# AI-sandbox/gnomix

Measured on AMD Instinct MI355X. Metric: haplotypes/sec (+ windows/sec) chr22 7-ancestry inference, higher is better.
Workload: dtype int8 x 7-digit fixed-point weights -> exact i32/i64 logits, f64 sigmoid (logistic base); f32 (tree smoother)

## Files before the change

### gnomix_amd/csrc/gnx_internal.h

```cpp
#pragma once
#include <hip/hip_runtime.h>
#include <stdint.h>
#include <algorithm>
#include <memory>
#include <string>
#include <vector>

#include "../../include/gnomix_hip.h"
#include "gnx_rank_table.h"

struct gnx_devbuf {
  void* p = nullptr;
  size_t cap = 0;
};

struct gnx_prof_pair {
  hipEvent_t a, b;
  int kid;
};

struct gnx_tune {
  int lr_bpc = 0, lr_want = 0;
  int lr_mt = 0, lr_waves = 0;
  int lr_flags = 0;
  int lr_dl = -1;
  int lr_nbuf = 0;
  int p2_mt = 0, p2_cw = 0, p2_ew = 0, p2_xsn = 0, p2_nbuf = 0;
  int p2_decline = 0;
  int lr_p2 = 1;
  int lr_flat = -1;
  int lr_w512 = 0;
  int lr_ws = 0, lr_ws_pw = 2;
  int sm_nw = 0;
  int sm_pair = 1;
  int smf_rpl = 0, smf_nw = 0;
  int crf_impl = 0;
  int crf_flags = 0;
  int forest_threads = 0;
  int forest_wrun = 0;
  int forest_halves = 0;
  int forest_impl = 0;
  int forest_flags = 0;
  int64_t host_batch = 0;
  int h2d_overlap = 1;
  int lr_lds_pad = 0, sm_lds_pad = 0;
  int gnofix_impl = 0;
  int gnofix_aux = 1;
  int gnofix_threads = 0;
  int debug = 0;
};

#define GNX_LDS_OPTIN(bytes, ...)                                                                                  \
  do {                                                                                                             \
    const hipError_t e_optin_ = hipFuncSetAttribute(reinterpret_cast<const void*>(&__VA_ARGS__),                   \
                                                    hipFuncAttributeMaxDynamicSharedMemorySize, (int)(bytes));     \
    if (e_optin_ != hipSuccess) return e_optin_;                                                                   \
  } while (0)

struct gnx_ctx {
  int device = 0;
  gnx_tune tune;
  hipStream_t stream = nullptr;
  bool own_stream = false;
  bool usable = false;
  std::string err;
  int n_cu = 256;
  gnx_devbuf ws_x, ws_b32, ws_b64, ws_p32, ws_p64, ws_lab, ws_misc, ws_scale, ws_bits, ws_lastrow, ws_rpair, ws_y0, ws_cal, ws_marg;
  hipStream_t s_aux = nullptr;
  hipEvent_t ev_aux[2] = {nullptr, nullptr};
  hipStream_t s_in = nullptr, s_out = nullptr;
  hipEvent_t ev_in[2] = {nullptr, nullptr}, ev_done[2] = {nullptr, nullptr}, ev_out[2] = {nullptr, nullptr};
  gnx_devbuf ws_pk, ws_xu, ws_xu2, ws_psi;
  gnx_devbuf ws_rank;
  gnx_devbuf ws_fb, ws_fb_body;
  gnx_devbuf ws_gt2, ws_src, ws_gt2o;
  bool prof = false;
  std::vector<gnx_prof_pair> prof_pending;
  std::vector<hipEvent_t> prof_pool;
  double prof_ms[GNX_K_COUNT] = {0};
  int64_t prof_n[GNX_K_COUNT] = {0};
};

struct BaseLRDev {
  const double* V = nullptr;
  const int8_t* V8 = nullptr;
  const int8_t* V8F = nullptr;
  const double* wscale = nullptr;
  const double* icpt = nullptr;
  const int32_t* chunk_j0 = nullptr;
  const int32_t* chunk_flush0 = nullptr;
  const int32_t* chunk_nflush = nullptr;
  const int32_t* win_chunk0 = nullptr;
  const int32_t* win_chunk1 = nullptr;
  int32_t n_chunks = 0;
  int32_t R = 0;
  int32_t NT = 0;
  int32_t NF = 0;
  int32_t max_piece_chunks = 0;
  const int8_t* V2 = nullptr;
  const int32_t* run_byte = nullptr;
  const int32_t* run_flush0 = nullptr;
  const int32_t* run_nflush = nullptr;
  const int32_t* win_run0 = nullptr;
  const int32_t* win_run1 = nullptr;
  int32_t n_runs = 0;
  int32_t EPR = 0;
  int32_t NT2 = 0;
  const int8_t* V2F = nullptr;
};
constexpr int GNX_LR_FLAT_COLS = 24;
constexpr int GNX_LR_FLAT_TILES = 11;
constexpr int GNX_LR_FLAT_MAX_SPAN = 84;

struct BaseLRLaunch {
  const int8_t* X;
  const int8_t* last_row;
  int64_t N, ldx;
  BaseLRDev d;
  const int32_t* h_win_chunk0;
  const int32_t* h_win_chunk1;
  int32_t W, A, wch;
  int32_t n_htiles;
  int32_t n_rg8;
  int32_t flags;
  int32_t max_chunks;
  int32_t max_wins;
  float* b32;
  double* b64;
  unsigned long long* dbg = nullptr;
};

struct SmoothXGBDev {
  const uint8_t* packed = nullptr;
  const int32_t* group_tree0 = nullptr;
  const int32_t* group_class = nullptr;
  int32_t n_groups = 0, n_trees = 0, D = 0, tree_bytes = 0, max_group = 0;
  float base_score = 0.5f;
  const uint8_t* rk_packed = nullptr;
  const float* rk_thr = nullptr;
  const GnxRankEntry* rk_lut = nullptr;
  const int32_t* rk_group_tree0 = nullptr;
  const int32_t* rk_group_class = nullptr;
  int32_t rk_K = 0, rk_steps = 0, rk_stride = 0, rk_tree_bytes = 0, rk_n_groups = 0, rk_max_group = 0;
  int32_t rk_bits = 0;
  int32_t rk_rpl = 0;
  const uint8_t* h8_packed = nullptr;
  const int32_t* h8_group_tree0 = nullptr;
  const int32_t* h8_group_class = nullptr;
  int32_t h8_tree_bytes = 0, h8_n_groups = 0, h8_max_group = 0;
  const uint8_t* rp_packed = nullptr;
  const int32_t* rp_group_tree0 = nullptr;
  const int32_t* rp_group_class = nullptr;
  int32_t rp_tree_bytes = 0, rp_n_groups = 0, rp_max_group = 0;
  int32_t impl = 0;
  const uint8_t* h3_packed = nullptr;
  const int32_t* h3_group_tree0 = nullptr;
  const int32_t* h3_group_class = nullptr;
  int32_t h3_n_groups = 0, h3_max_group = 0;
  const uint32_t* gf_packed = nullptr;
  int32_t gf_pitch = 0, gf_max_class = 0;
  const uint32_t* bs_nodes = nullptr;
  const float* bs_leaves = nullptr;
  const float* bs_thr = nullptr;
  const uint32_t* bs_lut = nullptr;
  const int32_t* bs_uoff = nullptr;
  const int32_t* bs_binoff = nullptr;
  const int32_t* bs_class_tree0 = nullptr;
  int32_t bs_steps = 0, bs_nbins = 0, bs_wc = 0, bs_nthr = 0, bs_maxbins = 0;
};

struct GnxBsLayout {
  int32_t wp, nr, rw, rb, nbins, hist_bytes, off_cnt, off_hist, off_P, off_bin, off_pi, off_seg, off_wtot, nseg, sl, total;
  uint32_t inv_sl;
};
GnxBsLayout gnx_bs_layout(int A, int S, int wc, int nbins);

__host__ __device__ inline int gnx_gf_tree_words(int D) { return 2 << D; }
constexpr int GNX_GF_PAD_TREES = 24;

constexpr int GNX_H32_WPB = 96;
constexpr int GNX_H32_TREE_BYTES = 320;
constexpr int GNX_H32_MAX_GROUP = 16;
inline size_t gnx_h32_lds_bytes(int A, int S, int G) {
  return (size_t)2 * G * GNX_H32_TREE_BYTES + (size_t)((GNX_H32_WPB + S) / 2) * A * 128;
}
constexpr int GNX_RK_RPL_MAX = 6;

static inline int gnx_tree_bytes(int D) {
  const int half = 1 << (D - 1);
  return ((half * 16 + (half - 1) * 8) + 15) & ~15;
}

#if defined(__HIPCC__)
__device__ __forceinline__ float gnx_walk(const uint8_t* tb, const uint8_t* row, int D) {
  const uint32_t half = 1u << (D - 1);
  uint32_t j = 1;
  for (int d = 0; d < D - 1; ++d) {
    uint2 nd;
    __builtin_memcpy(&nd, tb + half * 16 + (j - 1) * 8, 8);
    float fv;
    __builtin_memcpy(&fv, row + nd.x, 4);
    j = 2 * j + ((fv < __uint_as_float(nd.y)) ? 0u : 1u);
  }
  uint4 n4;
  __builtin_memcpy(&n4, tb + (j - half) * 16, 16);
  float fv;
  __builtin_memcpy(&fv, row + n4.x, 4);
  return (fv < __uint_as_float(n4.y)) ? __uint_as_float(n4.z) : __uint_as_float(n4.w);
}
#endif

struct SmoothXGBLaunch {
  const void* B;
  int32_t b_is_f64;
  int64_t N;
  int32_t W, A, S;
  SmoothXGBDev d;
  float* proba;
  float* marg;
  double* proba64;
  int32_t* labels;
};


struct SmoothCRFLaunch {
  const void* B;
  int32_t b_is_f64;
  int64_t N;
  int32_t W, A;
  const double* state;
  const double* etrans;
  double* psi;
  double* alpha;
  double* scale;
  double* proba64;
  float* proba32;
  int32_t* labels;
  int32_t norm_mask;
};

#ifdef GNX_EXPERIMENTS
hipError_t gnx_launch_smooth_crf_mm(const SmoothCRFLaunch& L, hipStream_t s);
hipError_t gnx_launch_smooth_crf_quad(const SmoothCRFLaunch& L, hipStream_t s);
#endif

struct SmoothCNNLaunch {
  const void* B;
  int32_t b_is_f64;
  int64_t N;
  int32_t W, A, S, reserved;
  const float* weight;
  const float* bias;
  float* proba32;
  double* proba64;
  int32_t* labels;
};

struct SvcWinDev {
  int32_t width, nw, n_sv, g_off;
  int32_t n_ms, poly;
  int64_t sv_off;
  int64_t coef_off;
  int32_t cls_start[36];
  int64_t rv_off;
  double poly_p;
};

struct CovRSKDev {
  const SvcWinDev* win = nullptr;
  const uint32_t* svbits = nullptr;
  const double* coef = nullptr;
  const uint32_t* gtab = nullptr;
  int32_t max_nw = 0, max_width = 0;
  std::vector<int32_t> fast_nw;
};

struct CovRSKLaunch {
  const uint32_t* planes;
  int64_t N, nwp, M;
  int32_t W, A;
  const SvcWinDev* win;
  const uint32_t* svbits;
  const double* coef;
  const uint32_t* gtab;
  int32_t max_nw, max_width;
  float* b32;
  double* b64;
  double* rpair;
  int64_t rpair_haps;
  int64_t n_first, n_count;
  int32_t w_first;
  const int32_t* host_fast_nw;
  hipStream_t aux;
  hipEvent_t ev_fork, ev_join;
  int32_t n_cu;
};

struct GnofixLaunch {
  int8_t* X;
  int64_t ldx, C;
  int32_t x_packed;
  const double* B;
  const int32_t* Y0;
  int32_t* Yout;
  int32_t* n_switches;
  int32_t W, A, S, max_it;
  SmoothXGBDev d;
  const int32_t* class_tree0;
  int32_t bp_in_lds;
  float* bp_scratch;
  uint32_t* hist;
  const uint16_t* R;
  const uint32_t* dif;
  uint32_t* par;
  const uint32_t* gf;
  const float* proba0;
  const float* pmax0;
  const int32_t* order;
  int32_t gf_pitch, gf_cap;
};

struct CalibMaps {
  const int32_t* off;
  const double* x;
  const double* y;
  int32_t thr_f32;
};
struct CalibLaunch {
  const void* in;
  int32_t in_is_f64;
  int64_t R;
  int32_t A;
  const int32_t* off;
  const double* x;
  const double* y;
  int32_t thr_f32;
  double* out64;
  float* out32;
// ... 192 lines not shown
```

### gnomix_amd/csrc/gnx_model_build.hip

```cpp
#include <algorithm>
#include <cmath>
#include <cstdio>
#include <cstdlib>
#include <cstring>
#include <limits>
#include <new>
#include <thread>
#include <utility>

#include "gnx_internal.h"

static inline int fail(gnx_ctx* ctx, int code, const std::string& msg) { return gnx_fail(ctx, code, msg); }

#define HIPCHK(ctx, expr)                                                                      \
  do {                                                                                         \
    hipError_t e__ = (expr);                                                                   \
    if (e__ != hipSuccess)                                                                     \
      return fail((ctx), GNX_EHIP, std::string(#expr) + ": " + hipGetErrorString(e__));        \
  } while (0)

template <typename F>
static unsigned parallel_ranges(size_t n, size_t grain, F&& fn) {
  unsigned nth = std::min<unsigned>(std::max(1u, std::thread::hardware_concurrency()), 16u);
  nth = (unsigned)std::min<size_t>(nth, std::max<size_t>(1, n / std::max<size_t>(grain, 1)));
// ... 430 lines not shown
      ll = d->cond[o + d->left[o + nid]];
      lr = d->cond[o + d->right[o + nid]];
    }
    uint8_t* p = out + (size_t)(j - half) * 16;
    std::memcpy(p, &foff, 4); std::memcpy(p + 4, &thr, 4); std::memcpy(p + 8, &ll, 4); std::memcpy(p + 12, &lr, 4);
    return;
  }
  uint32_t foff = 0;
  float thr = inf;
  if (!leaf) { foff = (uint32_t)d->feat[o + nid] * 4u; thr = d->cond[o + nid]; }
  uint8_t* p = out + (size_t)half * 16 + (size_t)(j - 1) * 8;
  std::memcpy(p, &foff, 4); std::memcpy(p + 4, &thr, 4);
  tree_fill(d, o, leaf ? nid : d->left[o + nid], 2 * j, depth + 1, D, out);
  tree_fill(d, o, leaf ? nid : d->right[o + nid], 2 * j + 1, depth + 1, D, out);
}

static void tree_fill_rk(const gnx_model_desc* d, int32_t o, int32_t nid, uint32_t j, int depth, int D,
                         const std::vector<float>& U, int stride, uint32_t* nodes, float* leaves) {
  const bool leaf = d->left[o + nid] == -1;
  if (depth == D) {
    leaves[j - (1u << D)] = d->cond[o + nid];
    return;
  }
  uint32_t word = 0xFFFFu << 16;
  if (!leaf) {
    const float thr = d->cond[o + nid];
    uint32_t field;
    if (thr != thr || thr == -std::numeric_limits<float>::infinity()) field = 0;
    else if (thr == std::numeric_limits<float>::infinity()) field = 0xFFFFu;
    else field = (uint32_t)(std::lower_bound(U.begin(), U.end(), thr) - U.begin()) + 1u;
    const int f = d->feat[o + nid], A = d->A;
    const uint32_t off = (uint32_t)(((f % A) * stride + f / A) * 2);
    word = (field << 16) | off;
  }
  nodes[j] = word;
  tree_fill_rk(d, o, leaf ? nid : d->left[o + nid], 2 * j, depth + 1, D, U, stride, nodes, leaves);
  tree_fill_rk(d, o, leaf ? nid : d->right[o + nid], 2 * j + 1, depth + 1, D, U, stride, nodes, leaves);
}

static int build_xgb_rk(gnx_model* m, const gnx_model_desc* d, const std::vector<int32_t>& order, int D) {
  const char* impl = std::getenv("GNX_SMOOTH_IMPL");
  if (impl && std::string(impl) == "f32") return GNX_OK;
  const int A = d->A, S = d->S;
  std::vector<float> U;
  for (int t = 0; t < d->n_trees; ++t)
    for (int32_t k = d->tree_off[t]; k < d->tree_off[t + 1]; ++k)
      if (d->left[k] != -1 && std::isfinite(d->cond[k])) U.push_back(d->cond[k]);
  std::sort(U.begin(), U.end());
  U.erase(std::unique(U.begin(), U.end()), U.end());
  const int nseg = (int)((d->C / d->M + 63) / 64);
  int rpl = 1;
  if (nseg >= 2) {
    int best_waste = 1 << 30;
    for (int r : {3, 2, 4}) {
      const int waste = (nseg + r - 1) / r * r - nseg;
      if (waste < best_waste) { best_waste = waste; rpl = r; }
    }
  }
  if (const char* e = std::getenv("GNX_RK_RPL")) rpl = std::max(1, std::min(GNX_RK_RPL_MAX, std::atoi(e)));
  int stride = rpl * 64 + S - 1;
  stride += stride & 1;
  if (U.size() > 65000 || (size_t)A * stride * 2 > 65535) return GNX_OK;
  if (U.empty()) U.push_back(0.5f);
  const int K = (int)U.size();
  GnxRankTable rt;
  gnx_rank_table_build(U, std::getenv("GNX_RK_BITS") ? std::atoi(std::getenv("GNX_RK_BITS")) : 0, rt);
  const std::vector<GnxRankEntry>& lut = rt.lut;
  const int steps = rt.steps;
  const int tree_bytes = 8 << D;
  int group_bytes = 4096;
  if (const char* e = std::getenv("GNX_RK_GROUP_BYTES")) group_bytes = std::max(tree_bytes, std::min(8192, std::atoi(e)));
  const int G = std::max(1, group_bytes / tree_bytes);
  std::vector<int32_t> group_tree0, group_class;
  {
    int in_group = 0, cur = -1;
    for (size_t k = 0; k < order.size(); ++k) {
      const int c = d->tree_class[order[k]];
      if (c != cur || in_group == G) { group_tree0.push_back((int32_t)k); group_class.push_back(c); in_group = 0; cur = c; }
      ++in_group;
    }
    group_tree0.push_back((int32_t)order.size());
  }
  std::vector<uint8_t> packed(order.size() * (size_t)tree_bytes, 0);
  for (size_t k = 0; k < order.size(); ++k) {
    uint8_t* tb = packed.data() + k * tree_bytes;
    tree_fill_rk(d, d->tree_off[order[k]], 0, 1, 0, D, U, stride, reinterpret_cast<uint32_t*>(tb),
                 reinterpret_cast<float*>(tb + ((size_t)4 << D)));
  }
  int rc;
  if ((rc = gnx_dev_upload(m, packed, &m->xgb.rk_packed, 64)) != GNX_OK) return rc;
  if ((rc = gnx_dev_upload(m, U, &m->xgb.rk_thr, 64)) != GNX_OK) return rc;
  if ((rc = gnx_dev_upload(m, lut, &m->xgb.rk_lut)) != GNX_OK) return rc;
  if ((rc = gnx_dev_upload(m, group_tree0, &m->xgb.rk_group_tree0)) != GNX_OK) return rc;
  if ((rc = gnx_dev_upload(m, group_class, &m->xgb.rk_group_class)) != GNX_OK) return rc;
  m->xgb.rk_K = K; m->xgb.rk_bits = rt.bits; m->xgb.rk_steps = steps; m->xgb.rk_stride = stride; m->xgb.rk_tree_bytes = tree_bytes;
  m->xgb.rk_n_groups = (int32_t)group_class.size(); m->xgb.rk_max_group = G; m->xgb.rk_rpl = rpl;
#ifdef GNX_EXPERIMENTS
  m->xgb.impl = (impl && std::string(impl) == "h64") ? 2 : (impl && std::string(impl) == "rk") ? 1 : 3;
#else
  m->xgb.impl = (impl && std::string(impl) == "rk") ? 1 : 3;
#endif
  if ((size_t)A * (2 * S + 2) * 2 <= 65535) {
    const int pitch = 2 * S + 2;
    const size_t tw = (size_t)gnx_gf_tree_words(D);
    std::vector<uint32_t> gf((order.size() + GNX_GF_PAD_TREES) * tw, 0u);
    for (size_t k = 0; k < order.size(); ++k) {
      uint32_t* tb = gf.data() + k * tw;
      tree_fill_rk(d, d->tree_off[order[k]], 0, 1, 0, D, U, pitch, tb, reinterpret_cast<float*>(tb + ((size_t)1 << D)));
    }
    if ((rc = gnx_dev_upload(m, gf, &m->xgb.gf_packed, 64)) != GNX_OK) return rc;
    std::vector<int> cnt(A, 0);
    int mc = 0;
    for (size_t k = 0; k < order.size(); ++k) mc = std::max(mc, ++cnt[d->tree_class[order[k]]]);
    m->xgb.gf_pitch = pitch; m->xgb.gf_max_class = mc;
  }
  if (D >= 2 && D <= 6) {
    const int tbp = 12 << D;
    const int Gp = std::max(2, (4096 / tbp) & ~1);
    std::vector<int32_t> gp_tree0, gp_class;
    {
      int in_group = 0, cur = -1;
      for (size_t k = 0; k < order.size(); ++k) {
        const int c = d->tree_class[order[k]];
        if (c != cur || in_group == Gp) { gp_tree0.push_back((int32_t)k); gp_class.push_back(c); in_group = 0; cur = c; }
        ++in_group;
      }
      gp_tree0.push_back((int32_t)order.size());
    }
    std::vector<uint8_t> pp(order.size() * (size_t)tbp, 0);
    std::vector<uint32_t> nodes((size_t)1 << D);
    std::vector<float> leaves((size_t)1 << D);
    size_t g = 0;
    for (size_t k = 0; k < order.size(); ++k) {
      while ((size_t)gp_tree0[g + 1] <= k) ++g;
      const uint32_t base = (uint32_t)(k - (size_t)gp_tree0[g]) * (uint32_t)tbp;
      std::fill(nodes.begin(), nodes.end(), 0u);
      tree_fill_rk(d, d->tree_off[order[k]], 0, 1, 0, D, U, stride, nodes.data(), leaves.data());
      uint32_t* o = reinterpret_cast<uint32_t*>(pp.data() + k * tbp);
      auto kids = [&](uint32_t j) {
        const uint32_t l = 2 * j < (1u << D) ? base + 8u * (2 * j) : base + (8u << D) + 4u * (2 * j - (1u << D));
        const uint32_t step = 2 * j < (1u << D) ? 8u : 4u;
        return l | ((l + step) << 16);
      };
      for (uint32_t j = 2; j < (1u << D); ++j) { o[2 * j] = nodes[j]; o[2 * j + 1] = kids(j); }
      o[0] = nodes[2]; o[1] = nodes[3]; o[2] = nodes[1]; o[3] = kids(2);
      memcpy(pp.data() + k * tbp + ((size_t)8 << D), leaves.data(), sizeof(float) << D);
    }
    if ((rc = gnx_dev_upload(m, pp, &m->xgb.rp_packed, 64)) != GNX_OK) return rc;
    if ((rc = gnx_dev_upload(m, gp_tree0, &m->xgb.rp_group_tree0)) != GNX_OK) return rc;
    if ((rc = gnx_dev_upload(m, gp_class, &m->xgb.rp_group_class)) != GNX_OK) return rc;
    m->xgb.rp_tree_bytes = tbp; m->xgb.rp_n_groups = (int32_t)gp_class.size(); m->xgb.rp_max_group = Gp;
  }
  if (D == 4 && ((size_t)(S >> 1) * A + A) * 128 <= 65536) {
    constexpr int tb3 = GNX_H32_TREE_BYTES;
    int G3 = 2;
    {
      const size_t strip = gnx_h32_lds_bytes(A, S, 0);
      if (strip + 4 * (size_t)tb3 <= (size_t)80 * 1024) G3 = std::min(GNX_H32_MAX_GROUP, (int)((((size_t)80 * 1024 - strip) / 2) / tb3) & ~1);
    }
    std::vector<int32_t> g3_tree0, g3_class;
    {
      int in_group = 0, cur = -1;
      for (size_t k = 0; k < order.size(); ++k) {
        const int c = d->tree_class[order[k]];
        if (c != cur || in_group == G3) { g3_tree0.push_back((int32_t)k); g3_class.push_back(c); in_group = 0; cur = c; }
        ++in_group;
      }
      g3_tree0.push_back((int32_t)order.size());
    }
    std::vector<uint8_t> p3(order.size() * (size_t)tb3, 0);
    std::vector<uint32_t> nodes(16);
    std::vector<float> leaves(16);
    size_t g = 0;
    for (size_t k = 0; k < order.size(); ++k) {
      while ((size_t)g3_tree0[g + 1] <= k) ++g;
      const uint32_t base = (uint32_t)(k - (size_t)g3_tree0[g]) * (uint32_t)tb3;
      std::fill(nodes.begin(), nodes.end(), 0u);
      tree_fill_rk(d, d->tree_off[order[k]], 0, 1, 0, 4, U, stride, nodes.data(), leaves.data());
      for (uint32_t odd = 0; odd < 2; ++odd) {
        const uint32_t nb = base + odd * 192u;
        uint32_t* o = reinterpret_cast<uint32_t*>(p3.data() + k * tb3 + odd * 192u);
        auto w0 = [&](uint32_t j) {
          const uint32_t hw = (nodes[j] & 0xffffu) / 2, a = hw / (uint32_t)stride, s = hw - a * (uint32_t)stride + odd;
          return (nodes[j] & 0xffff0000u) | (((s >> 1) * (uint32_t)A + a) * 128u + (s & 1u) * 2u);
        };
        auto kids = [&](uint32_t j) {
          const uint32_t l = 2 * j < 16u ? nb + 8u * (2 * j) : base + 128u + 4u * (2 * j - 16u);
          const uint32_t step = 2 * j < 16u ? 8u : 4u;
          return l | ((l + step) << 16);
        };
        for (uint32_t j = 2; j < 16u; ++j) { o[2 * j] = w0(j); o[2 * j + 1] = kids(j); }
        o[0] = w0(2); o[1] = w0(3); o[2] = w0(1); o[3] = kids(2);
      }
      memcpy(p3.data() + k * tb3 + 128, leaves.data(), 64);
    }
    if ((rc = gnx_dev_upload(m, p3, &m->xgb.h3_packed, 64)) != GNX_OK) return rc;
    if ((rc = gnx_dev_upload(m, g3_tree0, &m->xgb.h3_group_tree0)) != GNX_OK) return rc;
    if ((rc = gnx_dev_upload(m, g3_class, &m->xgb.h3_group_class)) != GNX_OK) return rc;
    m->xgb.h3_n_groups = (int32_t)g3_class.size(); m->xgb.h3_max_group = G3;
    if (!impl || !*impl) m->xgb.impl = 6;
    else if (std::string(impl) == "h32") m->xgb.impl = 5;
  }
#ifdef GNX_EXPERIMENTS
  if (D >= 2 && D <= 6 && (size_t)S * A < 65536) {
    const int tb8 = 12 << D;
    int G8 = std::max(4, (4096 / tb8) & ~3);
    {
      const size_t strip16 = (size_t)(16 * 3 + S - 1) * A * 128;
      if (strip16 + 2 * (size_t)G8 * tb8 <= (size_t)160 * 1024) {
        int per_class = 0;
        std::vector<int> cnt(A, 0);
        for (size_t k = 0; k < order.size(); ++k) per_class = std::max(per_class, ++cnt[d->tree_class[order[k]]]);
        const int fit = (int)((((size_t)160 * 1024 - strip16) / 2) / tb8) & ~3;
        G8 = std::max(G8, std::min({fit, (32768 / tb8) & ~3, (per_class + 3) & ~3}));
      }
    }
    std::vector<int32_t> g8_tree0, g8_class;
    {
      int in_group = 0, cur = -1;
      for (size_t k = 0; k < order.size(); ++k) {
        const int c = d->tree_class[order[k]];
        if (c != cur || in_group == G8) { g8_tree0.push_back((int32_t)k); g8_class.push_back(c); in_group = 0; cur = c; }
        ++in_group;
      }
      g8_tree0.push_back((int32_t)order.size());
    }
    std::vector<uint8_t> p8(order.size() * (size_t)tb8, 0);
    std::vector<uint32_t> nodes((size_t)1 << D);
    std::vector<float> leaves((size_t)1 << D);
    size_t g = 0;
    for (size_t k = 0; k < order.size(); ++k) {
      while ((size_t)g8_tree0[g + 1] <= k) ++g;
      const uint32_t base = (uint32_t)(k - (size_t)g8_tree0[g]) * (uint32_t)tb8;
      std::fill(nodes.begin(), nodes.end(), 0u);
      tree_fill_rk(d, d->tree_off[order[k]], 0, 1, 0, D, U, stride, nodes.data(), leaves.data());
      for (uint32_t j = 1; j < (1u << D); ++j) {
        const uint32_t h = (nodes[j] & 0xffffu) / 2, a = h / (uint32_t)stride, sidx = h - a * (uint32_t)stride;
        nodes[j] = (nodes[j] & 0xffff0000u) | (sidx * (uint32_t)A + a);
      }
      uint32_t* o = reinterpret_cast<uint32_t*>(p8.data() + k * tb8);
      auto kids = [&](uint32_t j) {
        const uint32_t l = 2 * j < (1u << D) ? base + 8u * (2 * j) : base + (8u << D) + 4u * (2 * j - (1u << D));
        const uint32_t step = 2 * j < (1u << D) ? 8u : 4u;
        return l | ((l + step) << 16);
      };
      for (uint32_t j = 2; j < (1u << D); ++j) { o[2 * j] = nodes[j]; o[2 * j + 1] = kids(j); }
      o[0] = nodes[2]; o[1] = nodes[3]; o[2] = nodes[1]; o[3] = kids(2);
      memcpy(p8.data() + k * tb8 + ((size_t)8 << D), leaves.data(), sizeof(float) << D);
    }
    if ((rc = gnx_dev_upload(m, p8, &m->xgb.h8_packed, 64)) != GNX_OK) return rc;
    if ((rc = gnx_dev_upload(m, g8_tree0, &m->xgb.h8_group_tree0)) != GNX_OK) return rc;
    if ((rc = gnx_dev_upload(m, g8_class, &m->xgb.h8_group_class)) != GNX_OK) return rc;
    m->xgb.h8_tree_bytes = tb8; m->xgb.h8_n_groups = (int32_t)g8_class.size(); m->xgb.h8_max_group = G8;
  }
#endif
  return GNX_OK;
}

#ifdef GNX_EXPERIMENTS
static void tree_fill_bs(const gnx_model_desc* d, int32_t o, int32_t nid, uint32_t j, int depth, const std::vector<std::vector<float>>& Uc,
                         const std::vector<int32_t>& binoff, const GnxBsLayout& Y, uint32_t* words, float* leaves) {
  const bool leaf = d->left[o + nid] == -1;
  if (depth == 4) {
    leaves[j - 16u] = d->cond[o + nid];
    return;
  }
  uint32_t a = 0, kf = 0, sw = 0;
  if (!leaf) {
    const float thr = d->cond[o + nid];
    const int f = d->feat[o + nid], A = d->A;
    a = (uint32_t)(f % A);
    sw = (uint32_t)(f / A);
    const std::vector<float>& U = Uc[a];
    if (thr != thr || thr == -std::numeric_limits<float>::infinity()) kf = 0;
    else if (thr == std::numeric_limits<float>::infinity()) kf = (uint32_t)U.size() + 1u;
    else kf = (uint32_t)(std::lower_bound(U.begin(), U.end(), thr) - U.begin()) + 1u;
  }
  const uint32_t cnt_addr = (uint32_t)Y.off_cnt + (uint32_t)binoff[a] + kf;
  words[2 * j] = (sw & 31u) | (cnt_addr << 16);
  words[2 * j + 1] = (uint32_t)Y.off_P + a * (uint32_t)(Y.nr * Y.rb) + (sw >> 5) * 4u;
  tree_fill_bs(d, o, leaf ? nid : d->left[o + nid], 2 * j, depth + 1, Uc, binoff, Y, words, leaves);
  tree_fill_bs(d, o, leaf ? nid : d->right[o + nid], 2 * j + 1, depth + 1, Uc, binoff, Y, words, leaves);
}

static int build_xgb_bs(gnx_model* m, const gnx_model_desc* d, const std::vector<int32_t>& order, int D) {
  const char* impl = std::getenv("GNX_SMOOTH_IMPL");
  if (impl && std::string(impl) == "f32") return GNX_OK;
  const int A = d->A, S = d->S;
  if (D > 4 || A > 16) return GNX_OK;
  std::vector<std::vector<float>> Uc((size_t)A);
  for (int t = 0; t < d->n_trees; ++t)
    for (int32_t k = d->tree_off[t]; k < d->tree_off[t + 1]; ++k)
      if (d->left[k] != -1 && std::isfinite(d->cond[k])) Uc[(size_t)(d->feat[k] % A)].push_back(d->cond[k]);
  std::vector<int32_t> uoff((size_t)A + 1, 0), binoff((size_t)A + 1, 0);
  std::vector<float> U;
  for (int c = 0; c < A; ++c) {
    std::vector<float>& u = Uc[(size_t)c];
    std::sort(u.begin(), u.end());
    u.erase(std::unique(u.begin(), u.end()), u.end());
    if (u.empty()) u.push_back(0.5f);
    if (u.size() > 60000) return GNX_OK;
    U.insert(U.end(), u.begin(), u.end());
    uoff[(size_t)c + 1] = (int32_t)U.size();
    binoff[(size_t)c + 1] = binoff[(size_t)c] + (((int32_t)u.size() + 2 + 15) & ~15);
  }
  const int nbins = binoff[(size_t)A];
  if (nbins > 65000) return GNX_OK;
  int wc = 128;
  if (wc + S - 1 > 255 || gnx_bs_layout(A, S, wc, nbins).total > 160 * 1024) return GNX_OK;
  const GnxBsLayout Y = gnx_bs_layout(A, S, wc, nbins);
  std::vector<uint32_t> lut((size_t)A * 1024);
  int steps = 0;
  for (int c = 0; c < A; ++c) {
    const std::vector<float>& u = Uc[(size_t)c];
    const int K = (int)u.size();
    for (int b = 0; b < 1024; ++b) {
      const int lo = b == 0 ? 0 : (int)(std::lower_bound(u.begin(), u.end(), (float)b / 1024.0f) - u.begin());
      const int hi = b == 1023 ? K : (int)(std::lower_bound(u.begin(), u.end(), (float)(b + 1) / 1024.0f) - u.begin());
      lut[(size_t)c * 1024 + (size_t)b] = (uint32_t)lo | ((uint32_t)hi << 16);
      int st = 0;
      while ((1 << st) < hi - lo + 1) ++st;
      steps = std::max(steps, st);
    }
  }
  std::vector<uint32_t> nodes(order.size() * 32, 0u);
  std::vector<float> leaves(order.size() * 16, 0.f);
  for (size_t k = 0; k < order.size(); ++k)
    tree_fill_bs(d, d->tree_off[order[k]], 0, 1, 0, Uc, binoff, Y, nodes.data() + k * 32, leaves.data() + k * 16);
  std::vector<int32_t> ct0((size_t)A + 1, 0);
  for (int t = 0; t < d->n_trees; ++t) ct0[(size_t)d->tree_class[t] + 1] += 1;
  for (int c = 0; c < A; ++c) ct0[(size_t)c + 1] += ct0[(size_t)c];
  int rc;
  if ((rc = gnx_dev_upload(m, nodes, &m->xgb.bs_nodes, 128)) != GNX_OK) return rc;
  if ((rc = gnx_dev_upload(m, leaves, &m->xgb.bs_leaves, 64)) != GNX_OK) return rc;
  if ((rc = gnx_dev_upload(m, U, &m->xgb.bs_thr, 64)) != GNX_OK) return rc;
  if ((rc = gnx_dev_upload(m, lut, &m->xgb.bs_lut)) != GNX_OK) return rc;
  if ((rc = gnx_dev_upload(m, uoff, &m->xgb.bs_uoff)) != GNX_OK) return rc;
  if ((rc = gnx_dev_upload(m, binoff, &m->xgb.bs_binoff)) != GNX_OK) return rc;
  if ((rc = gnx_dev_upload(m, ct0, &m->xgb.bs_class_tree0)) != GNX_OK) return rc;
  m->xgb.bs_steps = steps; m->xgb.bs_nbins = nbins; m->xgb.bs_wc = wc; m->xgb.bs_nthr = (int32_t)U.size();
  for (int c = 0; c < A; ++c) m->xgb.bs_maxbins = std::max(m->xgb.bs_maxbins, binoff[(size_t)c + 1] - binoff[(size_t)c]);
  if (impl && std::string(impl) == "bs") m->xgb.impl = 4;
  return GNX_OK;
}
#endif

int gnx_build_xgb(gnx_model* m, const gnx_model_desc* d) {
  gnx_ctx* ctx = m->ctx;
  const int A = d->A, S = d->S, F = S * A;
  if (d->n_trees <= 0 || !d->tree_off || !d->left || !d->right || !d->feat || !d->cond || !d->tree_class)
    return fail(ctx, GNX_EINVAL, "xgb smoother: tree arrays missing");
  const int64_t W = d->C / d->M;
// ... 385 lines not shown
```

### gnomix_amd/csrc/k_smooth_xgb_h32.hip

```cpp
#include <cstdio>
#include <cstdlib>

#include "gnx_internal.h"
#include "gnx_exp.h"
#include "gnx_rank.h"

namespace {

constexpr int HB = 32;
constexpr int RW = 3;
constexpr int NWAVE = 16;
constexpr int WPW = 2 * RW;
constexpr int WPB = NWAVE * WPW;
constexpr int THREADS = NWAVE * 64;
constexpr int TB = GNX_H32_TREE_BYTES;
static_assert(WPB == GNX_H32_WPB, "the model loader sizes the staging groups for this block");

#if defined(__HIP_DEVICE_COMPILE__)
template <typename T>
__device__ __forceinline__ const __attribute__((address_space(3))) T* lds_at(uint32_t a) {
  return (const __attribute__((address_space(3))) T*)(uintptr_t)a;
}
#else
template <typename T>
__device__ const T* lds_at(uint32_t) { return nullptr; }
#endif
typedef uint32_t u32x2 __attribute__((ext_vector_type(2)));
typedef uint32_t u32x4 __attribute__((ext_vector_type(4)));
__device__ __forceinline__ uint32_t step_ptr(uint32_t w0, uint32_t w1, uint32_t r) {
  uint32_t p;
  asm("v_cmp_le_u32_sdwa vcc, %[n], %[r] src0_sel:WORD_1 src1_sel:DWORD\n\t"
      "v_cndmask_b32_sdwa %[p], %[w], %[w], vcc dst_sel:DWORD dst_unused:UNUSED_PAD src0_sel:WORD_0 src1_sel:WORD_1"
      : [p] "=v"(p)
      : [n] "v"(w0), [r] "v"(r), [w] "v"(w1)
      : "vcc");
  return p;
}
__device__ __forceinline__ void first_ptr(uint32_t root, uint32_t r, uint32_t l0, uint32_t r0, uint32_t l1, uint32_t r1, uint32_t& w0,
                                          uint32_t& w1) {
  asm("v_cmp_le_u32_sdwa vcc, %[n], %[r] src0_sel:WORD_1 src1_sel:DWORD\n\t"
      "v_cndmask_b32 %[x], %[l0], %[r0], vcc\n\t"
      "v_cndmask_b32 %[y], %[l1], %[r1], vcc"
      : [x] "=&v"(w0), [y] "=&v"(w1)
      : [n] "v"(root), [r] "v"(r), [l0] "v"(l0), [r0] "v"(r0), [l1] "v"(l1), [r1] "v"(r1)
      : "vcc");
}

template <int NT>
__device__ __forceinline__ void walk_h32(uint32_t tb, const uint32_t* rb, float* psum) {
  constexpr int NC = NT * RW;
  uint32_t w0[NC], w1[NC], r[NC], p[NC];
  u32x4 top[NT];
#pragma unroll
  for (int t = 0; t < NT; ++t) top[t] = *lds_at<u32x4>(tb + t * TB);
  constexpr uint32_t SIB = 16u * 0x10001u;
#pragma unroll
  for (int c = 0; c < NC; ++c) r[c] = *lds_at<uint16_t>(rb[c % RW] + (top[c / RW].z & 0xffffu));
#pragma unroll
  for (int c = 0; c < NC; ++c)
    first_ptr(top[c / RW].z, r[c], top[c / RW].x, top[c / RW].y, top[c / RW].w, top[c / RW].w + SIB, w0[c], w1[c]);
#pragma unroll
  for (int c = 0; c < NC; ++c) r[c] = *lds_at<uint16_t>(rb[c % RW] + (w0[c] & 0xffffu));
#pragma unroll
  for (int c = 0; c < NC; ++c) p[c] = step_ptr(w0[c], w1[c], r[c]);
#pragma unroll
  for (int d = 2; d < 4; ++d) {
#pragma unroll
    for (int c = 0; c < NC; ++c) {
      const u32x2 nd = *lds_at<u32x2>(p[c]);
      w0[c] = nd.x;
      w1[c] = nd.y;
    }
#pragma unroll
    for (int c = 0; c < NC; ++c) r[c] = *lds_at<uint16_t>(rb[c % RW] + (w0[c] & 0xffffu));
#pragma unroll
    for (int c = 0; c < NC; ++c) p[c] = step_ptr(w0[c], w1[c], r[c]);
  }
  float lf[NC];
#pragma unroll
  for (int c = 0; c < NC; ++c) lf[c] = *lds_at<float>(p[c]);
#pragma unroll
  for (int t = 0; t < NT; ++t)
#pragma unroll
    for (int k = 0; k < RW; ++k) psum[k] += lf[t * RW + k];
}

__global__ __launch_bounds__(THREADS, 8) void k_smooth_xgb_h32(SmoothXGBLaunch L, int gw) {
  extern __shared__ __attribute__((aligned(16))) uint8_t lds[];
  const int A = L.A, W = L.W, S = L.S, pad = (S + 1) / 2;
  const int buf_bytes = L.d.h3_max_group * TB;
  const int P = WPB + S - 1;
  uint8_t* tbuf0 = lds;
  uint8_t* tbuf1 = tbuf0 + buf_bytes;
  uint8_t* strip = tbuf1 + buf_bytes;
  const int tid = threadIdx.x, lane = tid & 63, wave = tid >> 6, h = lane & 31, hv = lane >> 5;
  const int64_t hb = blockIdx.y, h0 = hb * HB;
  const int w0 = blockIdx.x * WPB;

  {
    constexpr int NV = 4;
    const int per_h = P * A;
    const int hl = (wave & 1) * 16 + (lane >> 2);
    const size_t row = (size_t)min(h0 + hl, L.N - 1) * W;
    const int dq = 32 / A, da = 32 - dq * A;
    int rr = (wave >> 1) * 4 + (lane & 3);
    int q = rr / A, a = rr - q * A;
    const bool interior = w0 >= pad && w0 + P <= pad + W;
    const size_t run0 = (row + (size_t)(interior ? w0 - pad : 0)) * A;
    for (; rr < per_h; rr += NV * 32) {
      float p[NV];
      uint32_t r[NV];
      int dst[NV];
      bool ok[NV];
      if (interior) {
#pragma unroll
        for (int i = 0; i < NV; ++i) {
          ok[i] = rr + i * 32 < per_h;
          const size_t idx = run0 + (size_t)min(rr + i * 32, per_h - 1);
          p[i] = L.b_is_f64 ? (float)reinterpret_cast<const double*>(L.B)[idx] : reinterpret_cast<const float*>(L.B)[idx];
          dst[i] = ((q >> 1) * A + a) * 128 + hl * 4 + (q & 1) * 2;
          a += da;
          q += dq;
          if (a >= A) { a -= A; ++q; }
        }
      } else {
#pragma unroll
        for (int i = 0; i < NV; ++i) {
          ok[i] = rr + i * 32 < per_h;
          const int qc = ok[i] ? q : P - 1, ac = ok[i] ? a : A - 1;
          const int j = min(w0 + qc, W + 2 * pad - 1);
          const size_t idx = (row + slide_src(j, W, pad)) * A + ac;
          p[i] = L.b_is_f64 ? (float)reinterpret_cast<const double*>(L.B)[idx] : reinterpret_cast<const float*>(L.B)[idx];
          dst[i] = ((qc >> 1) * A + ac) * 128 + hl * 4 + (qc & 1) * 2;
          a += da;
          q += dq;
          if (a >= A) { a -= A; ++q; }
        }
      }
      ranks<NV>(L.d.rk_thr, L.d.rk_lut, L.d.rk_K, L.d.rk_bits, L.d.rk_steps, p, r);
#pragma unroll
      for (int i = 0; i < NV; ++i)
        if (ok[i]) *reinterpret_cast<uint16_t*>(strip + dst[i]) = (uint16_t)r[i];
    }
  }

  const int64_t n = h0 + h;
  uint32_t rb[RW];
  bool valid[RW];
#pragma unroll
  for (int k = 0; k < RW; ++k) {
    rb[k] = (uint32_t)(uintptr_t)strip + (uint32_t)(((wave * RW + k) * A) * 128 + h * 4);
    valid[k] = (n < L.N) && (w0 + wave * WPW + 2 * k + hv < W);
  }
  const size_t cls_stride = (size_t)gridDim.y * W * HB;
  float* mrow = L.marg + ((size_t)hb * W + w0 + wave * WPW + hv) * HB + h;

  const int ng = L.d.h3_n_groups;
  uint4 stg;
#define GNX_G_LOAD(g)                                                                               \
  {                                                                                                 \
    const int t0_ = L.d.h3_group_tree0[g], t1_ = L.d.h3_group_tree0[(g) + 1];                       \
    const int last_ = (t1_ - t0_) * TB / 16 - 1;                                                    \
    stg = reinterpret_cast<const uint4*>(L.d.h3_packed + (size_t)t0_ * TB)[min(tid, last_)];        \
  }
#define GNX_G_STORE(dst)                                                                            \
  {                                                                                                 \
     \
    const int pc_ = (tid * 16 % TB) >> 4;                                                           \
    const bool node_ = pc_ < 8 || pc_ >= 12;                                                        \
    const uint32_t add_ = node_ ? (uint32_t)(uintptr_t)(dst) * 0x10001u : 0u;                       \
    stg.w += add_;                                                                                  \
    stg.y += (pc_ == 0 || pc_ == 12) ? 0u : add_;                                                   \
    if (tid * 16 < buf_bytes) *reinterpret_cast<uint4*>((dst) + (size_t)tid * 16) = stg;            \
  }
  float psum[RW];
#pragma unroll
  for (int k = 0; k < RW; ++k) psum[k] = 0.f;

  GNX_G_LOAD(0);
  GNX_G_STORE(tbuf0);
  __syncthreads();

  int cur_class = L.d.h3_group_class[0];
  for (int g = 0; g < ng; ++g) {
    uint8_t* cur = (g & 1) ? tbuf1 : tbuf0;
    uint8_t* nxt = (g & 1) ? tbuf0 : tbuf1;
    const int gn = min(g + 1, ng - 1);
    GNX_G_LOAD(gn);
    const int cls = L.d.h3_group_class[g];
    if (cls != cur_class) {
#pragma unroll
      for (int k = 0; k < RW; ++k) {
        if (valid[k]) mrow[(size_t)cur_class * cls_stride + (size_t)(2 * k) * HB] = L.d.base_score + psum[k];
        psum[k] = 0.f;
      }
      cur_class = cls;
    }
    const int nt = L.d.h3_group_tree0[g + 1] - L.d.h3_group_tree0[g];
    const uint32_t tb = (uint32_t)(uintptr_t)cur + (uint32_t)hv * 192u;
    int t = 0;
    for (; t + 2 <= nt; t += 2) walk_h32<2>(tb + (uint32_t)t * TB, rb, psum);
    for (; t < nt; ++t) walk_h32<1>(tb + (uint32_t)t * TB, rb, psum);
    GNX_G_STORE(nxt);
    __syncthreads();
  }
#undef GNX_G_LOAD
#undef GNX_G_STORE
#pragma unroll
  for (int k = 0; k < RW; ++k)
    if (valid[k]) mrow[(size_t)cur_class * cls_stride + (size_t)(2 * k) * HB] = L.d.base_score + psum[k];

  float* tile = reinterpret_cast<float*>(lds);
  const int rowlen = gw * WPW * A, pitch = rowlen | 1;
  for (int g0 = 0; g0 < NWAVE; g0 += gw) {
    if (wave >= g0 && wave < g0 + gw) {
#pragma unroll
      for (int k = 0; k < RW; ++k) {
        if (!valid[k]) continue;
        const float* mg = mrow + (size_t)(2 * k) * HB;
        float* o = tile + (size_t)h * pitch + ((wave - g0) * WPW + 2 * k + hv) * A;
        float wmax = mg[0];
        for (int a = 1; a < A; ++a) wmax = fmaxf(mg[(size_t)a * cls_stride], wmax);
        double wsum = 0.0;
        for (int a = 0; a < A; ++a) {
          const float e = gnx_softmax_exp(mg[(size_t)a * cls_stride] - wmax);
          o[a] = e;
          wsum += (double)e;
        }
        const float fs = (float)wsum;
        for (int a = 0; a < A; ++a) o[a] = o[a] / fs;
      }
    }
    __syncthreads();
    const int wb = w0 + g0 * WPW;
    for (int e = tid; e < HB * rowlen; e += THREADS) {
      const int hl = e / rowlen, c = e - hl * rowlen;
      const int64_t nn = h0 + hl;
      if (nn < L.N && wb + c / A < W) {
        const float p = tile[(size_t)hl * pitch + c];
        const size_t idx = ((size_t)nn * W + wb) * A + c;
        L.proba[idx] = p;
        if (L.proba64) L.proba64[idx] = (double)p;
      }
    }
    if (L.labels) {
      const int nwl = gw * WPW;
      for (int e = tid; e < HB * nwl; e += THREADS) {
        const int hl = e / nwl, wl = e - hl * nwl;
        const int64_t nn = h0 + hl;
        if (nn < L.N && wb + wl < W) {
          const float* o = tile + (size_t)hl * pitch + wl * A;
          int best = 0;
          float bv = -1.f;
          for (int a = 0; a < A; ++a) {
            const float p = o[a];
            if (p > bv) { bv = p; best = a; }
          }
          L.labels[(size_t)nn * W + wb + wl] = best;
        }
      }
    }
    __syncthreads();
  }
}

size_t lds_need(const SmoothXGBDev& d, int A, int S) { return gnx_h32_lds_bytes(A, S, d.h3_max_group); }

}

bool gnx_smooth_h32_fits(const SmoothXGBDev& d, int A, int S) {
  return d.h3_packed && d.rk_thr && d.D == 4 && lds_need(d, A, S) <= (size_t)80 * 1024;
}

hipError_t gnx_launch_smooth_xgb_h32(const SmoothXGBLaunch& L, hipStream_t s) {
  if (L.N <= 0) return hipSuccess;
  if (!gnx_smooth_h32_fits(L.d, L.A, L.S)) return hipErrorInvalidValue;
  const size_t lds = lds_need(L.d, L.A, L.S);
  int gw = NWAVE;
  while (gw > 1 && (size_t)HB * ((size_t)(gw * WPW * L.A) | 1) * 4 > lds) gw >>= 1;
  if ((size_t)HB * ((size_t)(gw * WPW * L.A) | 1) * 4 > lds) return hipErrorInvalidValue;
  const dim3 grid((unsigned)((L.W + WPB - 1) / WPB), (unsigned)((L.N + HB - 1) / HB));
  GNX_LDS_OPTIN(lds, k_smooth_xgb_h32);
  hipLaunchKernelGGL(k_smooth_xgb_h32, grid, dim3(THREADS), lds, s, L, gw);
  return hipGetLastError();
}
```

Baseline: 3.731 million.

## Prebake LDS addresses into fixed-size h32 tree groups and skip dead waves

Tree packing moves to a shared header and pads each tree group to a fixed G-tree buffer. Child addresses are now baked at build time against absolute LDS offsets that alternate between two buffers. This removes the per-group address patching during staging and the loads of group start indices, and the staging load becomes a single strided read. Waves whose windows lie past the edge skip the tree walks, and the strip size uses only the live window count. The change relies on dynamic LDS starting at address zero (checked at runtime) and adds compile-time ablation switches, with some host memory spent on padding.

```diff
diff --git a/gnomix_amd/csrc/gnx_h32_layout.h b/gnomix_amd/csrc/gnx_h32_layout.h
--- /dev/null
+++ b/gnomix_amd/csrc/gnx_h32_layout.h
@@ -0,0 +1,75 @@
+#pragma once
+#include <stdint.h>
+#include <string.h>
+
+#include <algorithm>
+#include <vector>
+
+#if defined(__HIPCC__)
+#define GNX_H32_HD __host__ __device__ __forceinline__
+#else
+#define GNX_H32_HD inline
+#endif
+
+constexpr int GNX_H32_WPB = 96;
+constexpr int GNX_H32_TREE_BYTES = 320;
+constexpr int GNX_H32_MAX_GROUP = 16;
+
+GNX_H32_HD uint32_t gnx_h32_buf_bytes(int G) { return (uint32_t)G * (uint32_t)GNX_H32_TREE_BYTES; }
+GNX_H32_HD uint32_t gnx_h32_group_lds(int g, int G) { return (uint32_t)(g & 1) * gnx_h32_buf_bytes(G); }
+inline size_t gnx_h32_lds_bytes(int A, int S, int G) {
+  return (size_t)2 * gnx_h32_buf_bytes(G) + (size_t)((GNX_H32_WPB + S) / 2) * A * 128;
+}
+inline int gnx_h32_group_trees(int A, int S) {
+  const size_t strip = gnx_h32_lds_bytes(A, S, 0), tb = GNX_H32_TREE_BYTES;
+  if (strip + 4 * tb > (size_t)80 * 1024) return 2;
+  return std::min(GNX_H32_MAX_GROUP, (int)((((size_t)80 * 1024 - strip) / 2) / tb) & ~1);
+}
+
+struct GnxH32Pack {
+  int G = 0;
+  std::vector<int32_t> tree0, cls;
+  std::vector<uint8_t> packed;
+};
+
+inline void gnx_h32_pack(const std::vector<int>& cls, const std::vector<uint32_t>& nodes, const std::vector<float>& leaves, int A,
+                         int S, int stride, GnxH32Pack& out) {
+  constexpr uint32_t TB = GNX_H32_TREE_BYTES;
+  const int G = gnx_h32_group_trees(A, S);
+  out.G = G;
+  out.tree0.clear();
+  out.cls.clear();
+  {
+    int in_group = 0, cur = -1;
+    for (size_t k = 0; k < cls.size(); ++k) {
+      if (cls[k] != cur || in_group == G) { out.tree0.push_back((int32_t)k); out.cls.push_back(cls[k]); in_group = 0; cur = cls[k]; }
+      ++in_group;
+    }
+    out.tree0.push_back((int32_t)cls.size());
+  }
+  out.packed.assign(out.cls.size() * (size_t)gnx_h32_buf_bytes(G), 0);
+  size_t g = 0;
+  for (size_t k = 0; k < cls.size(); ++k) {
+    while ((size_t)out.tree0[g + 1] <= k) ++g;
+    const uint32_t in_group = (uint32_t)(k - (size_t)out.tree0[g]);
+    const uint32_t base = gnx_h32_group_lds((int)g, G) + in_group * TB;
+    uint8_t* tree = out.packed.data() + g * (size_t)gnx_h32_buf_bytes(G) + (size_t)in_group * TB;
+    const uint32_t* nd = nodes.data() + 16 * k;
+    for (uint32_t odd = 0; odd < 2; ++odd) {
+      const uint32_t nb = base + odd * 192u;
+      uint32_t* o = reinterpret_cast<uint32_t*>(tree + odd * 192u);
+      auto w0 = [&](uint32_t j) {
+        const uint32_t hw = (nd[j] & 0xffffu) / 2, a = hw / (uint32_t)stride, s = hw - a * (uint32_t)stride + odd;
+        return (nd[j] & 0xffff0000u) | (((s >> 1) * (uint32_t)A + a) * 128u + (s & 1u) * 2u);
+      };
+      auto kids = [&](uint32_t j) {
+        const uint32_t l = 2 * j < 16u ? nb + 8u * (2 * j) : base + 128u + 4u * (2 * j - 16u);
+        const uint32_t step = 2 * j < 16u ? 8u : 4u;
+        return l | ((l + step) << 16);
+      };
+      for (uint32_t j = 2; j < 16u; ++j) { o[2 * j] = w0(j); o[2 * j + 1] = kids(j); }
+      o[0] = w0(2); o[1] = w0(3); o[2] = w0(1); o[3] = kids(2);
+    }
+    memcpy(tree + 128, leaves.data() + 16 * k, 64);
+  }
+}
diff --git a/gnomix_amd/csrc/gnx_internal.h b/gnomix_amd/csrc/gnx_internal.h
--- a/gnomix_amd/csrc/gnx_internal.h
+++ b/gnomix_amd/csrc/gnx_internal.h
@@ -8,6 +8,7 @@
 
 #include "../../include/gnomix_hip.h"
 #include "gnx_rank_table.h"
+#include "gnx_h32_layout.h"
 
 struct gnx_devbuf {
   void* p = nullptr;
@@ -178,12 +179,6 @@
 __host__ __device__ inline int gnx_gf_tree_words(int D) { return 2 << D; }
 constexpr int GNX_GF_PAD_TREES = 24;
 
-constexpr int GNX_H32_WPB = 96;
-constexpr int GNX_H32_TREE_BYTES = 320;
-constexpr int GNX_H32_MAX_GROUP = 16;
-inline size_t gnx_h32_lds_bytes(int A, int S, int G) {
-  return (size_t)2 * G * GNX_H32_TREE_BYTES + (size_t)((GNX_H32_WPB + S) / 2) * A * 128;
-}
 constexpr int GNX_RK_RPL_MAX = 6;
 
 static inline int gnx_tree_bytes(int D) {
diff --git a/gnomix_amd/csrc/gnx_model_build.hip b/gnomix_amd/csrc/gnx_model_build.hip
--- a/gnomix_amd/csrc/gnx_model_build.hip
+++ b/gnomix_amd/csrc/gnx_model_build.hip
@@ -606,52 +606,19 @@
     m->xgb.rp_tree_bytes = tbp; m->xgb.rp_n_groups = (int32_t)gp_class.size(); m->xgb.rp_max_group = Gp;
   }
   if (D == 4 && ((size_t)(S >> 1) * A + A) * 128 <= 65536) {
-    constexpr int tb3 = GNX_H32_TREE_BYTES;
-    int G3 = 2;
-    {
-      const size_t strip = gnx_h32_lds_bytes(A, S, 0);
-      if (strip + 4 * (size_t)tb3 <= (size_t)80 * 1024) G3 = std::min(GNX_H32_MAX_GROUP, (int)((((size_t)80 * 1024 - strip) / 2) / tb3) & ~1);
-    }
-    std::vector<int32_t> g3_tree0, g3_class;
-    {
-      int in_group = 0, cur = -1;
-      for (size_t k = 0; k < order.size(); ++k) {
-        const int c = d->tree_class[order[k]];
-        if (c != cur || in_group == G3) { g3_tree0.push_back((int32_t)k); g3_class.push_back(c); in_group = 0; cur = c; }
-        ++in_group;
-      }
-      g3_tree0.push_back((int32_t)order.size());
-    }
-    std::vector<uint8_t> p3(order.size() * (size_t)tb3, 0);
-    std::vector<uint32_t> nodes(16);
-    std::vector<float> leaves(16);
-    size_t g = 0;
+    std::vector<int> cls3(order.size());
+    std::vector<uint32_t> nodes(order.size() * 16, 0u);
+    std::vector<float> leaves(order.size() * 16, 0.f);
     for (size_t k = 0; k < order.size(); ++k) {
-      while ((size_t)g3_tree0[g + 1] <= k) ++g;
-      const uint32_t base = (uint32_t)(k - (size_t)g3_tree0[g]) * (uint32_t)tb3;
-      std::fill(nodes.begin(), nodes.end(), 0u);
-      tree_fill_rk(d, d->tree_off[order[k]], 0, 1, 0, 4, U, stride, nodes.data(), leaves.data());
-      for (uint32_t odd = 0; odd < 2; ++odd) {
-        const uint32_t nb = base + odd * 192u;
-        uint32_t* o = reinterpret_cast<uint32_t*>(p3.data() + k * tb3 + odd * 192u);
-        auto w0 = [&](uint32_t j) {
-          const uint32_t hw = (nodes[j] & 0xffffu) / 2, a = hw / (uint32_t)stride, s = hw - a * (uint32_t)stride + odd;
-          return (nodes[j] & 0xffff0000u) | (((s >> 1) * (uint32_t)A + a) * 128u + (s & 1u) * 2u);
-        };
-        auto kids = [&](uint32_t j) {
-          const uint32_t l = 2 * j < 16u ? nb + 8u * (2 * j) : base + 128u + 4u * (2 * j - 16u);
-          const uint32_t step = 2 * j < 16u ? 8u : 4u;
-          return l | ((l + step) << 16);
-        };
-        for (uint32_t j = 2; j < 16u; ++j) { o[2 * j] = w0(j); o[2 * j + 1] = kids(j); }
-        o[0] = w0(2); o[1] = w0(3); o[2] = w0(1); o[3] = kids(2);
-      }
-      memcpy(p3.data() + k * tb3 + 128, leaves.data(), 64);
-    }
-    if ((rc = gnx_dev_upload(m, p3, &m->xgb.h3_packed, 64)) != GNX_OK) return rc;
-    if ((rc = gnx_dev_upload(m, g3_tree0, &m->xgb.h3_group_tree0)) != GNX_OK) return rc;
-    if ((rc = gnx_dev_upload(m, g3_class, &m->xgb.h3_group_class)) != GNX_OK) return rc;
-    m->xgb.h3_n_groups = (int32_t)g3_class.size(); m->xgb.h3_max_group = G3;
+      cls3[k] = d->tree_class[order[k]];
+      tree_fill_rk(d, d->tree_off[order[k]], 0, 1, 0, 4, U, stride, nodes.data() + 16 * k, leaves.data() + 16 * k);
+    }
+    GnxH32Pack pk;
+    gnx_h32_pack(cls3, nodes, leaves, A, S, stride, pk);
+    if ((rc = gnx_dev_upload(m, pk.packed, &m->xgb.h3_packed, 64)) != GNX_OK) return rc;
+    if ((rc = gnx_dev_upload(m, pk.tree0, &m->xgb.h3_group_tree0)) != GNX_OK) return rc;
+    if ((rc = gnx_dev_upload(m, pk.cls, &m->xgb.h3_group_class)) != GNX_OK) return rc;
+    m->xgb.h3_n_groups = (int32_t)pk.cls.size(); m->xgb.h3_max_group = pk.G;
     if (!impl || !*impl) m->xgb.impl = 6;
     else if (std::string(impl) == "h32") m->xgb.impl = 5;
   }
diff --git a/gnomix_amd/csrc/k_smooth_xgb_h32.hip b/gnomix_amd/csrc/k_smooth_xgb_h32.hip
--- a/gnomix_amd/csrc/k_smooth_xgb_h32.hip
+++ b/gnomix_amd/csrc/k_smooth_xgb_h32.hip
@@ -5,8 +5,13 @@
 #include "gnx_exp.h"
 #include "gnx_rank.h"
 
+#ifndef GNX_H32_ABLATE
+#define GNX_H32_ABLATE 0
+#endif
+
 namespace {
 
+constexpr bool ABL_GROUPS = (GNX_H32_ABLATE & 3) != 0, ABL_BARRIER = (GNX_H32_ABLATE & 2) != 0;
 constexpr int HB = 32;
 constexpr int RW = 3;
 constexpr int NWAVE = 16;
@@ -24,6 +29,11 @@
 #else
 template <typename T>
 __device__ const T* lds_at(uint32_t) { return nullptr; }
+#endif
+#if defined(__HIP_DEVICE_COMPILE__)
+__device__ __forceinline__ int wave_uniform(int v) { return __builtin_amdgcn_readfirstlane(v); }
+#else
+__device__ int wave_uniform(int v) { return v; }
 #endif
 typedef uint32_t u32x2 __attribute__((ext_vector_type(2)));
 typedef uint32_t u32x4 __attribute__((ext_vector_type(4)));
@@ -88,14 +98,14 @@
 __global__ __launch_bounds__(THREADS, 8) void k_smooth_xgb_h32(SmoothXGBLaunch L, int gw) {
   extern __shared__ __attribute__((aligned(16))) uint8_t lds[];
   const int A = L.A, W = L.W, S = L.S, pad = (S + 1) / 2;
-  const int buf_bytes = L.d.h3_max_group * TB;
-  const int P = WPB + S - 1;
-  uint8_t* tbuf0 = lds;
-  uint8_t* tbuf1 = tbuf0 + buf_bytes;
-  uint8_t* strip = tbuf1 + buf_bytes;
+  const int G = L.d.h3_max_group;
+  const int buf_bytes = (int)gnx_h32_buf_bytes(G);
+  uint8_t* strip = lds + 2 * buf_bytes;
   const int tid = threadIdx.x, lane = tid & 63, wave = tid >> 6, h = lane & 31, hv = lane >> 5;
   const int64_t hb = blockIdx.y, h0 = hb * HB;
   const int w0 = blockIdx.x * WPB;
+  const int live = min(WPB, W - w0);
+  const int P = live + S - 1;
 
   {
     constexpr int NV = 4;
@@ -156,37 +166,22 @@
   float* mrow = L.marg + ((size_t)hb * W + w0 + wave * WPW + hv) * HB + h;
 
   const int ng = L.d.h3_n_groups;
-  uint4 stg;
-#define GNX_G_LOAD(g)                                                                               \
-  {                                                                                                 \
-    const int t0_ = L.d.h3_group_tree0[g], t1_ = L.d.h3_group_tree0[(g) + 1];                       \
-    const int last_ = (t1_ - t0_) * TB / 16 - 1;                                                    \
-    stg = reinterpret_cast<const uint4*>(L.d.h3_packed + (size_t)t0_ * TB)[min(tid, last_)];        \
-  }
-#define GNX_G_STORE(dst)                                                                            \
-  {                                                                                                 \
-     \
-    const int pc_ = (tid * 16 % TB) >> 4;                                                           \
-    const bool node_ = pc_ < 8 || pc_ >= 12;                                                        \
-    const uint32_t add_ = node_ ? (uint32_t)(uintptr_t)(dst) * 0x10001u : 0u;                       \
-    stg.w += add_;                                                                                  \
-    stg.y += (pc_ == 0 || pc_ == 12) ? 0u : add_;                                                   \
-    if (tid * 16 < buf_bytes) *reinterpret_cast<uint4*>((dst) + (size_t)tid * 16) = stg;            \
-  }
+  const uint32_t lds0 = (uint32_t)(uintptr_t)lds;
+  const bool stager = tid * 16 < buf_bytes;
+  const uint32_t piece = (uint32_t)min(tid * 16, buf_bytes - 16);
+  const bool wave_live = wave_uniform(wave) * WPW < live;
   float psum[RW];
 #pragma unroll
   for (int k = 0; k < RW; ++k) psum[k] = 0.f;
 
-  GNX_G_LOAD(0);
-  GNX_G_STORE(tbuf0);
+  uint4 stg = *reinterpret_cast<const uint4*>(L.d.h3_packed + piece);
+  if (stager) *reinterpret_cast<uint4*>(lds + gnx_h32_group_lds(0, G) + tid * 16) = stg;
   __syncthreads();
 
   int cur_class = L.d.h3_group_class[0];
   for (int g = 0; g < ng; ++g) {
-    uint8_t* cur = (g & 1) ? tbuf1 : tbuf0;
-    uint8_t* nxt = (g & 1) ? tbuf0 : tbuf1;
     const int gn = min(g + 1, ng - 1);
-    GNX_G_LOAD(gn);
+    if (!ABL_GROUPS) stg = *reinterpret_cast<const uint4*>(L.d.h3_packed + (size_t)gn * (size_t)buf_bytes + piece);
     const int cls = L.d.h3_group_class[g];
     if (cls != cur_class) {
 #pragma unroll
@@ -196,16 +191,18 @@
       }
       cur_class = cls;
     }
-    const int nt = L.d.h3_group_tree0[g + 1] - L.d.h3_group_tree0[g];
-    const uint32_t tb = (uint32_t)(uintptr_t)cur + (uint32_t)hv * 192u;
-    int t = 0;
-    for (; t + 2 <= nt; t += 2) walk_h32<2>(tb + (uint32_t)t * TB, rb, psum);
-    for (; t < nt; ++t) walk_h32<1>(tb + (uint32_t)t * TB, rb, psum);
-    GNX_G_STORE(nxt);
-    __syncthreads();
-  }
-#undef GNX_G_LOAD
-#undef GNX_G_STORE
+    int nt = L.d.h3_group_tree0[g + 1] - L.d.h3_group_tree0[g];
+    if (ABL_GROUPS) nt = min(nt, L.d.h3_group_tree0[1]);
+    if (wave_live) {
+      const uint32_t tb = lds0 + gnx_h32_group_lds(ABL_GROUPS ? 0 : g, G) + (uint32_t)hv * 192u;
+      int t = 0;
+      for (; t + 2 <= nt; t += 2) walk_h32<2>(tb + (uint32_t)t * TB, rb, psum);
+      for (; t < nt; ++t) walk_h32<1>(tb + (uint32_t)t * TB, rb, psum);
+    }
+    if (!ABL_GROUPS && stager) *reinterpret_cast<uint4*>(lds + gnx_h32_group_lds(g + 1, G) + tid * 16) = stg;
+    if (!ABL_BARRIER) __syncthreads();
+  }
+  if (ABL_BARRIER) __syncthreads();
 #pragma unroll
   for (int k = 0; k < RW; ++k)
     if (valid[k]) mrow[(size_t)cur_class * cls_stride + (size_t)(2 * k) * HB] = L.d.base_score + psum[k];
@@ -266,10 +263,18 @@
 
 size_t lds_need(const SmoothXGBDev& d, int A, int S) { return gnx_h32_lds_bytes(A, S, d.h3_max_group); }
 
+bool dynamic_lds_starts_at_zero() {
+  static const bool ok = [] {
+    hipFuncAttributes fa;
+    return hipFuncGetAttributes(&fa, reinterpret_cast<const void*>(k_smooth_xgb_h32)) == hipSuccess && fa.sharedSizeBytes == 0;
+  }();
+  return ok;
+}
+
 }
 
 bool gnx_smooth_h32_fits(const SmoothXGBDev& d, int A, int S) {
-  return d.h3_packed && d.rk_thr && d.D == 4 && lds_need(d, A, S) <= (size_t)80 * 1024;
+  return d.h3_packed && d.rk_thr && d.D == 4 && lds_need(d, A, S) <= (size_t)80 * 1024 && dynamic_lds_starts_at_zero();
 }
 
 hipError_t gnx_launch_smooth_xgb_h32(const SmoothXGBLaunch& L, hipStream_t s) {
```

After: 3.722 million, median of 2. Within noise of the previous version (-0.2%).
